# Xiaoming-Zhao/PointNav-VO

Hardware: AMD Instinct MI355X
Metric: RGB-D frame-pair VO inferences/s @341x192 (higher is better)
Workload: dtype f32

## Files before the change

### include/pnvo.h

```cpp
#ifndef PNVO_H_
#define PNVO_H_

#include <stddef.h>
#include <stdint.h>

#ifdef __cplusplus
extern "C" {
#endif

#define PNVO_OK 0
#define PNVO_ERR_ARG (-1)
#define PNVO_ERR_HIP (-2)
#define PNVO_ERR_STATE (-3)
#define PNVO_ERR_WEIGHTS (-4)
#define PNVO_ERR_INPUT (-5)

typedef struct pnvo_model_s *pnvo_handle;

typedef struct {
  int32_t width, height;
  int32_t n_rgb, n_depth, n_dd, n_tdv;
  int32_t baseplanes;
  int32_t hidden;
  int32_t out_dim;
// ... 124 lines not shown
int pnvo_policy_load_weights(pnvo_policy_handle h, const float *blob, size_t n_floats, const pnvo_tensor_desc *toc,
                             int ntoc);

int pnvo_policy_act(pnvo_policy_handle h, const float *depth, const float *goal, const int64_t *prev_actions,
                    const float *masks, const float *hidden_in, int B, float *hidden_out, float *features, float *logits,
                    float *value, void *stream);

int pnvo_policy_destroy(pnvo_policy_handle h);

int pnvo_avgpool2(const float *depth, int N, int H, int W, float *out, void *stream);

const char *pnvo_last_error(pnvo_handle h);

const char *pnvo_last_note(pnvo_handle h);


int pnvo_set_tap(pnvo_handle h, const char *name, float *dst, size_t capacity);
int pnvo_tap_shape(pnvo_handle h, const char *name, int B, int64_t shape[4]);

typedef struct {
  char name[96];
  int64_t launches;
  double total_ms;
  double flops;
  double bytes;
} pnvo_kernel_time;
int pnvo_forward_features(pnvo_handle h, const float *rgb, const float *depth, const float *dd, const float *tdv,
                          const int64_t *actions, int B, float *hidden_out, void *stream);

int pnvo_check_inputs(pnvo_handle h);

int pnvo_layer_kernel(pnvo_handle h, const char *name, int B, char *family, size_t cap, double *executed_flops);

int pnvo_timing_mode(pnvo_handle h, int mode);
int pnvo_timing_read(pnvo_handle h, pnvo_kernel_time *entries, int cap, int *n_out);

size_t pnvo_packed_conv_floats(int cout, int cin, int kh, int kw);
int pnvo_pack_conv_weight(const float *oihw, int cout, int cin, int kh, int kw, float *out);

int pnvo_resize_area(const void *src, int src_dtype, int n, int in_h, int in_w, int channels, int64_t src_frame_stride,
                     int64_t src_row_stride, int64_t src_pix_stride, int rs_h, int rs_w, int crop_y, int crop_x, int out_h, int out_w,
                     float *dst, int dst_group, int64_t dst_group_stride, int64_t dst_member_stride, int64_t dst_row_stride,
                     int64_t dst_pix_stride, int div_rule, void *stream);

const char *pnvo_version(void);

#ifdef __cplusplus
}
#endif
#endif
```

### pointnav-vo_amd/_lib.py

```python
import ctypes as C
import os

import torch

_HERE = os.path.dirname(os.path.abspath(__file__))
LIB_PATH = os.path.join(_HERE, "csrc", "libpnvo.so")

PNVO_OK = 0


GRAD_READY_FN = C.CFUNCTYPE(None, C.c_void_p, C.c_uint64, C.c_uint64, C.c_void_p)


class PnvoError(RuntimeError):
    pass


class pnvo_config(C.Structure):
    _fields_ = [(n, C.c_int32) for n in (
        "width", "height", "n_rgb", "n_depth", "n_dd", "n_tdv", "baseplanes", "hidden", "out_dim", "normalize",
        "act_embed", "n_acts", "flat_size", "max_batch", "backbone_depth")]


class pnvo_tensor_desc(C.Structure):
# ... 35 lines not shown
    "pnvo_dataset_pairs": (C.c_int, [C.c_void_p] * 7 + [C.c_int] * 5 + [C.c_void_p] * 7),
    "pnvo_topdown_view_pairs": (C.c_int, [C.c_void_p, C.c_int, C.c_int, C.c_int, C.POINTER(C.c_float), C.c_int, C.c_void_p, C.c_void_p,
                                          C.c_void_p]),
    "pnvo_topdown_view": (C.c_int, [C.c_void_p, C.c_int, C.c_int, C.c_int, C.c_int64, C.c_int64,
                                    C.POINTER(C.c_float), C.c_int, C.c_void_p, C.c_int64, C.c_int64, C.c_void_p,
                                    C.c_void_p]),
    "pnvo_train_attach": (C.c_int, [C.c_void_p, C.c_void_p, C.c_void_p, C.c_size_t, C.POINTER(pnvo_tensor_desc), C.c_int]),
    "pnvo_train_refresh": (C.c_int, [C.c_void_p, C.c_void_p]),
    "pnvo_train_forward": (C.c_int, [C.c_void_p, C.c_void_p, C.c_void_p, C.c_void_p, C.c_void_p, C.c_int, C.c_void_p,
                                     C.c_void_p, C.c_void_p, C.c_void_p]),
    "pnvo_train_backward": (C.c_int, [C.c_void_p, C.c_void_p, C.c_void_p]),
    "pnvo_train_set_grad_hook": (C.c_int, [C.c_void_p, C.c_void_p, C.c_void_p]),
    "pnvo_train_grad_buckets": (C.c_int, [C.c_void_p, C.POINTER(C.c_uint64), C.POINTER(C.c_uint64), C.c_int, C.POINTER(C.c_int)]),
    "pnvo_input_moments": (C.c_int, [C.c_void_p, C.c_void_p, C.c_void_p, C.c_void_p, C.c_void_p, C.c_int, C.c_void_p,
                                     C.c_int, C.c_void_p, C.c_void_p]),
    "pnvo_rmv_merge": (C.c_int, [C.c_void_p, C.c_int, C.c_int, C.c_void_p, C.c_void_p, C.c_void_p, C.c_void_p]),
    "pnvo_train_set_actions": (C.c_int, [C.c_void_p, C.c_void_p]),
    "pnvo_mse_loss": (C.c_int, [C.c_void_p, C.c_void_p, C.c_int, C.c_int, C.c_void_p, C.c_void_p, C.c_void_p]),
    "pnvo_mse_loss_coef": (C.c_int, [C.c_void_p, C.c_void_p, C.c_void_p, C.c_int, C.c_void_p, C.c_void_p, C.c_void_p]),
    "pnvo_geo_inverse_loss": (C.c_int, [C.c_void_p, C.c_void_p, C.c_int, C.c_int, C.c_float, C.c_void_p, C.c_void_p,
                                        C.c_void_p]),
    "pnvo_train_set_dropout": (C.c_int, [C.c_void_p, C.c_float, C.c_uint64]),
    "pnvo_train_dropout_mask": (C.c_int, [C.c_void_p, C.c_int, C.c_void_p, C.c_void_p]),
    "pnvo_adam_step": (C.c_int, [C.c_void_p, C.c_void_p, C.c_void_p, C.c_void_p, C.c_size_t, C.c_float, C.c_float,
                                 C.c_float, C.c_float, C.c_int, C.c_void_p]),
    "pnvo_destroy": (C.c_int, [C.c_void_p]),
    "pnvo_ring_assemble": (C.c_int, [C.c_void_p, C.c_void_p, C.c_void_p, C.c_void_p, C.c_void_p, C.c_void_p, C.c_void_p, C.c_int, C.c_int,
                                     C.c_int, C.c_void_p, C.c_void_p, C.c_void_p, C.c_void_p]),
    "pnvo_last_error": (C.c_char_p, [C.c_void_p]),
    "pnvo_last_note": (C.c_char_p, [C.c_void_p]),
    "pnvo_set_tap": (C.c_int, [C.c_void_p, C.c_char_p, C.c_void_p, C.c_size_t]),
    "pnvo_tap_shape": (C.c_int, [C.c_void_p, C.c_char_p, C.c_int, C.POINTER(C.c_int64)]),
    "pnvo_check_inputs": (C.c_int, [C.c_void_p]),
    "pnvo_forward_features": (C.c_int, [C.c_void_p, C.c_void_p, C.c_void_p, C.c_void_p, C.c_void_p, C.c_void_p, C.c_int,
                                        C.c_void_p, C.c_void_p]),
    "pnvo_policy_create": (C.c_int, [C.c_void_p, C.c_int, C.POINTER(C.c_void_p)]),
    "pnvo_policy_load_weights": (C.c_int, [C.c_void_p, C.c_void_p, C.c_size_t, C.c_void_p, C.c_int]),
    "pnvo_policy_act": (C.c_int, [C.c_void_p, C.c_void_p, C.c_void_p, C.c_void_p, C.c_void_p, C.c_void_p, C.c_int,
                                  C.c_void_p, C.c_void_p, C.c_void_p, C.c_void_p, C.c_void_p]),
    "pnvo_policy_destroy": (C.c_int, [C.c_void_p]),
    "pnvo_avgpool2": (C.c_int, [C.c_void_p, C.c_int, C.c_int, C.c_int, C.c_void_p, C.c_void_p]),
    "pnvo_layer_kernel": (C.c_int, [C.c_void_p, C.c_char_p, C.c_int, C.c_char_p, C.c_size_t, C.POINTER(C.c_double)]),
    "pnvo_timing_mode": (C.c_int, [C.c_void_p, C.c_int]),
    "pnvo_timing_read": (C.c_int, [C.c_void_p, C.POINTER(pnvo_kernel_time), C.c_int, C.POINTER(C.c_int)]),
    "pnvo_packed_conv_floats": (C.c_size_t, [C.c_int, C.c_int, C.c_int, C.c_int]),
    "pnvo_pack_conv_weight": (C.c_int, [C.c_void_p, C.c_int, C.c_int, C.c_int, C.c_int, C.c_void_p]),
    "pnvo_resize_area": (C.c_int, [C.c_void_p, C.c_int, C.c_int, C.c_int, C.c_int, C.c_int, C.c_int64, C.c_int64, C.c_int64,
                                   C.c_int, C.c_int, C.c_int, C.c_int, C.c_int, C.c_int, C.c_void_p, C.c_int, C.c_int64, C.c_int64,
                                   C.c_int64, C.c_int64, C.c_int, C.c_void_p]),
    "pnvo_version": (C.c_char_p, []),
}


def _load():
    if not os.path.exists(LIB_PATH):
        raise PnvoError(
            f"{LIB_PATH} is missing: the HIP extension has not been built.  Run "
            "`python -c 'import __graft_entry__ as g; g.build()'` (or `make -C pointnav-vo_amd/csrc`).  "
            "There is no CPU fallback.")
    lib = C.CDLL(LIB_PATH)
    for name, (res, args) in _SIGNATURES.items():
        fn = getattr(lib, name)
        fn.restype = res
        fn.argtypes = args
    return lib

# ... 13 lines not shown
```

### pointnav-vo_amd/csrc/pnvo_api.hip

```cpp
#include <hip/hip_runtime.h>

#include <cmath>
#include <cstdio>
#include <cstdlib>
#include <cstring>
#include <functional>
#include <atomic>
#include <condition_variable>
#include <map>
#include <mutex>
#include <string>
#include <thread>
#include <vector>

#include "pnvo_model.h"

using namespace pnvo;

thread_local std::string g_err;

int pnvo_fail(pnvo_handle h, int code, const std::string &msg) {
  if (h) h->err = msg;
  g_err = msg;
  return code;
// ... 578 lines not shown
  xa.y = r.y;
  xa.in_scale = r.in_scale;
  xa.in_shift = r.in_shift;
  xa.stats = m->stats;
  if (r.tail != nullptr) {
    if (r.in_scale == nullptr) return fail(m, PNVO_ERR_STATE, "block tail without the conv's GroupNorm scale/shift");
    xa.xout = r.tail->out;
  }
  const long P = (long)l.hout * l.wout;
  const int cpg = l.groups > 0 ? l.cout / l.groups : 0;
  const bool fuse = m->opt.gn_fuse && xa.slots == 1 && l.cout == l.coutp && cpg >= 1 && cpg <= 32 &&
                    32 % cpg == 0 && l.cout % cpg == 0 && (rows || !(xa.persist_wgs > 0 && l.cin == 32 && l.coutp == 32));
  if (fuse && ride != nullptr) {
    xa.ds_gamma = ride->cd->gamma;
    xa.ds_beta = ride->cd->beta;
    xa.ds_scale = ride->ss[0];
    xa.ds_shift = ride->ss[1];
    xa.ds_mu = ride->mu;
    xa.ds_rstd = ride->rstd;
  }
  if (fuse) {
    xa.gn_gamma = l.gamma;
    xa.gn_beta = l.beta;
    xa.gn_scale = r.ss[0];
    xa.gn_shift = r.ss[1];
    xa.gn_mu = r.mu;
    xa.gn_rstd = r.rstd;
    xa.gn_cpg = cpg;
    xa.gn_eps = 1e-5f;
    xa.gn_P = P;
  }
  {
    Timed t(m, s, "conv:" + l.name, conv_flops(l, B), conv_bytes(l, B) + (r.tail ? 8.0 * B * l.hin * l.win * l.cin : 0.0));
    if (rows)
      HIPCHK(m, launch_conv_rows32(xa, x3_mode, m->num_cus, s));
    else
      HIPCHK(m, launch_conv_x3(xa, l.k, l.stride, x3_mode, mw, nw, ldsb, s));
  }
  if (fuse) return PNVO_OK;
  Timed t(m, s, "gn_finalize", 0.0, 0.0);
  if (ride != nullptr) {
    const float *st2[2] = {m->stats, m->stats_ds}, *ga2[2] = {l.gamma, ride->cd->gamma}, *be2[2] = {l.beta, ride->cd->beta};
    float *sc2[2] = {r.ss[0], ride->ss[0]}, *sh2[2] = {r.ss[1], ride->ss[1]};
    float *mu2[2] = {r.mu, ride->mu}, *rs2[2] = {r.rstd, ride->rstd};
    HIPCHK(m, launch_gn_finalize_pair(st2, B, xa.slots, l.coutp, l.cout, l.groups, P, ga2, be2, 1e-5f, sc2, sh2, mu2, rs2, s,
                                      r.grp ? &gg : nullptr, r.grp ? &ggd : nullptr));
    return PNVO_OK;
  }
  HIPCHK(m, launch_gn_finalize(m->stats, B, xa.slots, l.coutp, l.cout, l.groups, P, 1, l.gamma, l.beta, 1e-5f, r.ss[0], r.ss[1], s,
                               xa.slots, r.mu, r.rstd, r.grp ? &gg : nullptr));
  return PNVO_OK;
}

int run_conv_fp32(pnvo_handle m, const Layer &l, int B, const ConvRequest &r) {
  hipStream_t s = r.s;
  ConvArgs a;
  conv_geometry(l, B, r.y_cstride, a);
  if (r.src != nullptr) {
    const int nsrc[4] = {m->cfg.n_rgb, m->cfg.n_depth, m->cfg.n_dd, m->cfg.n_tdv};
    a.src_mode = 1;
    a.zero_page = m->zero_page;
    for (int j = 0; j < m->CP / 8; ++j)
      for (int hh = 0; hh < 2; ++hh)
        for (int q = 0; q < 2; ++q) {
          const int nc = 8 * j + 4 * hh + 2 * q;
          const int tn = m->stem_tensor_of_new[nc];
          SrcPiece &pc = a.pieces[j][hh][q];
// ... 45 lines not shown
      a.kpart = m->kpart;
      a.ksplit = ks;
    }
  }
  {
    Timed t(m, s, "conv:" + l.name, conv_flops(l, B), conv_bytes(l, B));
    HIPCHK(m, launch_conv(a, s));
    if (a.ksplit > 1 && r.head_out != nullptr && P == 1 && r.y_cstride == l.cout) {
      HIPCHK(m, launch_ksplit_reduce_head(a, r.head_w, m->head_bias, m->cfg.out_dim, r.head_out, s));
      if (r.head_rode != nullptr) *r.head_rode = true;
    } else if (a.ksplit > 1) {
      HIPCHK(m, launch_ksplit_reduce(a, s));
    }
  }
  if (r.ss) {
    Timed t(m, s, "gn_finalize", 0.0, 0.0);
    HIPCHK(m, launch_gn_finalize(m->stats, B, a.slots, l.coutp, l.cout, l.groups, P, a.MT * 32, l.gamma, l.beta, 1e-5f,
                                 r.ss[0], r.ss[1], s, 0, r.mu, r.rstd));
  }
  return PNVO_OK;
}
}

int pnvo_run_conv(pnvo_handle m, const Layer &l, int B, const ConvRequest &r) {
  if (r.ss && r.src == nullptr && r.bias == nullptr && !r.relu_out && r.y_cstride == l.coutp && x3_layer(m, l)) {
    ConvX3Args xa;
    x3_fill(m, l, B, xa);
    if (r.tail != nullptr) {
      xa.res = r.tail->res;
      xa.res_scale = r.tail->res_scale;
      xa.res_shift = r.tail->res_shift;
    }
    const int x3_mode = r.tail ? (r.tail->res ? 2 : 3) : (r.in_scale ? 1 : 0);
    const bool rows = xa.np == 2 && m->opt.x3_rows && conv_rows32_plan(xa, l.k, l.stride, x3_mode, m->num_cus);
    int mw = 0, nw = 0;
    size_t ldsb = 0;
    if (rows || conv_x3_plan(xa, l.k, l.stride, &mw, &nw, &ldsb)) return run_conv_x3(m, l, B, r, xa, rows, x3_mode, mw, nw, ldsb);
  }
  if (r.tail != nullptr) return fail(m, PNVO_ERR_STATE, "block tail handed to a conv that cannot take it (" + l.name + ")");
  if (r.grp != nullptr && r.ss != nullptr) return fail(m, PNVO_ERR_STATE, "grouped forward: layer " + l.name + " fell off the float16-piece tile kernel");
  return run_conv_fp32(m, l, B, r);
}

StemPlan pnvo_stem_plan(pnvo_handle m, bool train_fwd, const RawFrames &raw) {
  const Layer &stem = m->convs[0];
  StemPlan p;
  p.lds_serves = (m->CPL <= 32) && (stem.coutp == 32 || stem.coutp == 64) && stem.cout == stem.coutp;
  const bool keeps_place = !m->dense_sticky || (!train_fwd && p.lds_serves);
  if (keeps_place && m->mx_ok && (!train_fwd || m->train_mx) && m->opt.stem <= 1)
    p.kernel = StemPlan::MX;
  else if (keeps_place && m->dd_ok && m->opt.stem != 3)
    p.kernel = StemPlan::DD;
  else
    p.kernel = p.lds_serves ? StemPlan::LDS : StemPlan::GENERIC;
  const bool fused = p.kernel == StemPlan::MX || p.kernel == StemPlan::DD;
  p.standin = fused && m->dense_sticky;
  p.slots = stem_slots(m, p.kernel);
  const bool on_device = m->opt.input_fallback && m->dd_flag != nullptr && !train_fwd && p.lds_serves;
  p.repairs = fused && !p.standin && raw.depth == nullptr && on_device;
  p.marks = m->dd_flag != nullptr && !m->dense_sticky && raw.depth == nullptr && !on_device;
  const bool loaded_current = m->train == nullptr || m->weights_gen == m->weights_gen_at_load;
  const bool h2_current = m->mx_wpk2_dev || (train_fwd ? m->train == nullptr : loaded_current);
  const bool want2 = train_fwd ? m->opt.train_pieces == 2 : m->opt.pieces == 2;
  p.pieces = (want2 && h2_current && m->mx_wpk2 != nullptr) ? 2 : 3;
  p.h2_from_host = m->opt.pieces == 2 && m->mx_wpk2 != nullptr && loaded_current;
  return p;
}
// ... 1530 lines not shown
    int hh = h->Hp, ww = h->Wp;
    for (int k = 1; k < li; ++k) {
      hh = halve(hh);
      ww = halve(ww);
    }
    return set(B, hh, ww, c.baseplanes << (li - 1));
  }
  return fail(h, PNVO_ERR_ARG, "unknown tap '" + n + "'");
}

int pnvo_layer_kernel(pnvo_handle h, const char *name, int B, char *family, size_t cap, double *executed_flops) {
  if (!h || !name || !family || cap == 0 || B <= 0) return fail(h, PNVO_ERR_ARG, "bad argument");
  for (size_t li = 1; li < h->convs.size(); ++li) {
    const Layer &l = h->convs[li];
    if (l.name != name) continue;
    const double alg = 2.0 * B * l.hout * l.wout * (double)l.cout * l.cin * l.k * l.kw;
    if (pnvo_stem_plan(h, false, {}).writes_slots() && pnvo_small_usable(h, B)) {
      std::snprintf(family, cap, "smallnet");
      if (executed_flops) {
        const int mb = l.cinp >= 128 ? 1 : l.cinp >= 64 ? 2 : 4, th = mb == 4 ? 8 : 4, tw = mb == 1 ? 4 : 8;
        *executed_flops = 2.0 * B * ((l.hout + th - 1) / th) * ((l.wout + tw - 1) / tw) * (th * tw) * (double)rup(l.cout, 16) * l.cinp * l.k * l.kw;
      }
      return PNVO_OK;
    }
    ConvX3Args xa;
    int mw, nw;
    size_t ldsb;
    if (l.k == 1 && l.stride == 2 && li >= 3 && h->convs[li - 2].stride == 2 && pnvo_conv_takes_ds(h, h->convs[li - 2], l, B) &&
        x3_args(h, h->convs[li - 2], B, xa, &mw, &nw, &ldsb)) {
      std::snprintf(family, cap, "x2-rides");
      if (executed_flops) *executed_flops = 3.0 * 2.0 * (double)B * xa.tiles_r * xa.tiles_c * xa.MT * 32.0 * l.coutp * (double)l.cinp;
      return PNVO_OK;
    }
    if (x3_layer(h, l) && l.groups > 0 && x3_args(h, l, B, xa, &mw, &nw, &ldsb)) {
      std::snprintf(family, cap, xa.np == 2 ? "x2" : "x3");
      if (executed_flops)
        *executed_flops = (xa.np == 2 ? 3.0 : 6.0) * 2.0 * (double)B * xa.tiles_r * xa.tiles_c * xa.MT * 32.0 * l.coutp * (double)l.cinp * l.k * l.kw;
      return PNVO_OK;
    }
    std::snprintf(family, cap, "%s", layer_on_lds(h, l, nullptr) ? "fp32-lds" : "fp32-generic");
    if (executed_flops) *executed_flops = alg;
    return PNVO_OK;
  }
  return fail(h, PNVO_ERR_ARG, std::string("no residual-stage conv named '") + name + "'");
}

int pnvo_timing_mode(pnvo_handle h, int mode) {
  if (!h) return fail(h, PNVO_ERR_ARG, "null handle");
  h->timing = mode ? 1 : 0;
  return PNVO_OK;
}

int pnvo_timing_read(pnvo_handle h, pnvo_kernel_time *entries, int cap, int *n_out) {
  if (!h || !n_out) return fail(h, PNVO_ERR_ARG, "null argument");
  for (auto &r : h->trecs) {
    HIPCHK(h, hipEventSynchronize(r.b));
    float ms = 0.f;
    HIPCHK(h, hipEventElapsedTime(&ms, r.a, r.b));
    h->tentries[r.entry].total_ms += ms;
    h->evpool.push_back(r.a);
    h->evpool.push_back(r.b);
  }
  h->trecs.clear();
  const int n = (int)h->tentries.size();
  *n_out = n;
  for (int k = 0; k < n && k < cap && entries; ++k) entries[k] = h->tentries[k];
  h->tentries.clear();
  h->tindex.clear();
  return PNVO_OK;
}

size_t pnvo_packed_conv_floats(int cout, int cin, int kh, int kw) { return packed_conv_floats(cout, cin, kh, kw); }

int pnvo_pack_conv_weight(const float *oihw, int cout, int cin, int kh, int kw, float *out) {
  if (!oihw || !out || cout <= 0 || cin <= 0 || kh <= 0 || kw <= 0) return fail(nullptr, PNVO_ERR_ARG, "bad argument");
  pack_conv_weight(oihw, cout, cin, kh, kw, out);
  return PNVO_OK;
// ... 4 lines not shown
```

### pointnav-vo_amd/csrc/pnvo_internal.h

```cpp
#pragma once
#include <mutex>
#include <hip/hip_runtime.h>
#include <stdint.h>

namespace pnvo {

constexpr int PNVO_ABSMAX_UINTS = 64 * 16;

struct SrcPiece {
  const float *base;
  int nch;
  int choff;
};

struct ConvArgs {
  const float *x;
  const float *wpk;
  float *y;
  const float *in_scale;
  const float *in_shift;
  float *stats;
  const float *bias;
  const int64_t *bias_row;
  int B, H, W, CIN;
// ... 132 lines not shown
  float *ds_scale, *ds_shift;
  float *ds_mu, *ds_rstd;
  int grp_end0, grp_end1;
  const unsigned short *wpk_g[2], *ds_wpk_g[2];
  float oscale_g[2], ds_oscale_g[2];
  const float *gn_gamma_g[2], *gn_beta_g[2], *ds_gamma_g[2], *ds_beta_g[2];
};
#if defined(__HIPCC__)
__device__ __forceinline__ void gn_finalize_lane(float s1, float s2, int cpg, long P, float eps, float gamma, float beta, float *scale, float *shift,
                                                 float *mu_out = nullptr, float *rstd_out = nullptr) {
#pragma clang fp contract(off)
  double d1 = (double)s1, d2 = (double)s2;
  for (int o = cpg >> 1; o >= 1; o >>= 1) {
    d1 += __shfl_xor(d1, o);
    d2 += __shfl_xor(d2, o);
  }
  const double cnt = (double)P * cpg;
  const double mu = d1 / cnt;
  double var = d2 / cnt - mu * mu;
  if (var < 0.0) var = 0.0;
  const double rstd = 1.0 / sqrt(var + (double)eps);
  if (mu_out != nullptr) {
    *mu_out = (float)mu;
    *rstd_out = (float)rstd;
  }
  const double sc = rstd * (double)gamma;
  *scale = (float)sc;
  *shift = (float)((double)beta - mu * sc);
}
#endif
bool conv_x3_plan(ConvX3Args &a, int ks, int stride, int *mw, int *nw, size_t *lds_bytes);
bool conv_rows32_plan(ConvX3Args &a, int ks, int stride, int mode, int num_cus);
hipError_t launch_conv_rows32(const ConvX3Args &a, int mode, int num_cus, hipStream_t s);
hipError_t launch_conv_x3(const ConvX3Args &a, int ks, int stride, int mode, int mw, int nw, size_t lds_bytes, hipStream_t s);
hipError_t launch_conv_x3_repack(const float *w_oihw, int cout, int cin, int cinp, int coutp, int kh, int kw, int transposed,
                                 unsigned short *out, hipStream_t s);
void pack_conv_x3_weight(const float *oihw, int cout, int cin, int cinp, int coutp, int kh, int kw, unsigned short *out);
hipError_t launch_conv_x2_scales(const float *params, const long *seg_dev, int nseg, float *out, hipStream_t s);
hipError_t launch_conv_x2_repack(const float *w_oihw, int cout, int cin, int cinp, int coutp, int kh, int kw, const float *scale_dev,
                                 unsigned short *out, hipStream_t s, int transposed = 0);
float pack_conv_x2_weight(const float *oihw, int cout, int cin, int cinp, int coutp, int kh, int kw, unsigned short *out);

struct ConvBArgs {
  const unsigned short *x[2];
  const unsigned short *wpk[2];
  void *y[2];
  const float *in_scale[2], *in_shift[2];
  const unsigned short *x2[2];
  const float *in_scale2[2], *in_shift2[2];
  unsigned short *xout[2];
  float *stats[2];
  int B, H, W, CIN, Ho, Wo, COUTP;
  int TR, TC, tiles_r, tiles_c, PR, PC, CK, MT, wn, slots;
  int persist_wgs;
  const unsigned short *ds_wpk[2];
  void *ds_y[2];
  float *ds_stats[2];
  const float *ds_gamma[2], *ds_beta[2];
  float *ds_scale[2], *ds_shift[2];
  const float *gn_gamma[2], *gn_beta[2];
  float *gn_scale[2], *gn_shift[2];
  int gn_cpg;
  float gn_eps;
  long gn_P;
};
bool conv_bf16_plan(ConvBArgs &a, int ks, int stride, int *mw, int *nw, size_t *lds_bytes);
// ... 200 lines not shown
```

### pointnav-vo_amd/vo_cnn.py

```python
import ctypes as C
import math

import numpy as np
import torch
import torch.nn as nn

from . import _lib
from . import model_spec as ms
from .common_vars import DEFAULT_DELTA_STATE_SIZE, N_ACTS, TOP_DOWN_VIEW_PAIR_CHANNEL
from .registry import baseline_registry


class _Holder(nn.Module):
    """Anonymous container so dotted state_dict names resolve exactly as in the reference module tree."""


def _init_tensor(name, shape, fan_in=None):
    t = torch.empty(shape)
    if len(shape) == 4 or (len(shape) == 2 and name != "action_embedding.weight"):
        if name == "output_head.1.weight":
            nn.init.orthogonal_(t)
        else:
            nn.init.kaiming_uniform_(t, a=math.sqrt(5))
    elif name == "action_embedding.weight":
# ... 244 lines not shown
            _lib.check(_lib.lib.pnvo_forward_raw(self._handle, p_rgb, p_dep, p_tdv, act_ptr, int(B), C.c_void_p(out.data_ptr()),
                                                 C.c_void_p(err_flag.data_ptr()) if err_flag is not None else None,
                                                 C.c_void_p(stream)), self._handle)
        return out

    def tap(self, name, observation_pairs, actions=None):
        dev = next(self.parameters()).device
        self._ensure_handle(dev)
        first = next(v for v in observation_pairs.values())
        B = first.shape[0]
        shape = (C.c_int64 * 4)()
        _lib.check(_lib.lib.pnvo_tap_shape(self._handle, name.encode(), int(B), shape), self._handle)
        buf = torch.empty(tuple(int(s) for s in shape), device=dev, dtype=torch.float32)
        _lib.check(_lib.lib.pnvo_set_tap(self._handle, name.encode(), C.c_void_p(buf.data_ptr()), buf.numel()),
                   self._handle)
        try:
            out = self.forward(observation_pairs, actions)
        finally:
            _lib.lib.pnvo_set_tap(self._handle, None, None, 0)
        return out, buf

    def check_inputs(self):
        if self._handle is not None:
            _lib.check(_lib.lib.pnvo_check_inputs(self._handle), self._handle)

    def layer_kernel(self, name, batch):
        dev = next(self.parameters()).device
        self._ensure_handle(dev)
        self._sync_weights()
        buf, fl = C.create_string_buffer(32), C.c_double(0.0)
        _lib.check(_lib.lib.pnvo_layer_kernel(self._handle, name.encode(), int(batch), buf, 32, C.byref(fl)), self._handle)
        return buf.value.decode(), float(fl.value)

    def timing(self, enable):
        dev = next(self.parameters()).device
        self._ensure_handle(dev)
        _lib.check(_lib.lib.pnvo_timing_mode(self._handle, int(bool(enable))), self._handle)

    def timing_read(self):
        ent = (_lib.pnvo_kernel_time * 128)()
        n = C.c_int(0)
        _lib.check(_lib.lib.pnvo_timing_read(self._handle, ent, 128, C.byref(n)), self._handle)
        return [dict(name=ent[i].name.decode(), launches=int(ent[i].launches), total_ms=float(ent[i].total_ms),
                     flops=float(ent[i].flops), bytes=float(ent[i].bytes)) for i in range(min(n.value, 128))]


def _obs_ptrs(model, observation_pairs, dev):
    c = model.cfg
    ptrs, B, keep = [], None, []
    for key, n in (("rgb", c.n_rgb), ("depth", c.n_depth), ("discretized_depth", c.n_dd), ("top_down_view", c.n_tdv)):
        if n == 0:
            ptrs.append(None)
            continue
        t = observation_pairs[key]
        if t.device != dev:
            raise RuntimeError(f"observation '{key}' is on {t.device}, model on {dev}")
        t = t.to(torch.float32).contiguous()
        if t.dim() != 4 or t.shape[1] != c.height or t.shape[2] != c.width or t.shape[3] != n:
            raise ValueError(f"observation '{key}' has shape {tuple(t.shape)}, expected [B,{c.height},{c.width},{n}]")
        B = t.shape[0] if B is None else B
        assert t.shape[0] == B
        keep.append(t)
        ptrs.append(C.c_void_p(t.data_ptr()))
    return ptrs, B, keep


# ... 146 lines not shown
```

Before: 114,300.

## Add 64-channel row-streaming MFMA conv kernel with DMA-to-LDS staging

Adds a specialized persistent row-streaming 3x3 conv kernel for 64-input-channel layers. Two wave sets alternate between MFMA compute and staging. Staging issues buffer loads directly into an LDS ring, applies GroupNorm scale/shift, ReLU and the residual, and splits values into fp16 hi/lo pairs. The dispatcher routes eligible inference layers to it instead of the 32-row kernel, and a run_layer API is added for testing single layers. It trades higher LDS use and register pressure for overlap of load, convert and compute, and applies only to inference paths without training or grouping.

New measurement: 115,400, median of 5. 1.01x the previous value.

```diff
diff --git a/include/pnvo.h b/include/pnvo.h
--- a/include/pnvo.h
+++ b/include/pnvo.h
@@ -180,6 +180,10 @@
 
 int pnvo_layer_kernel(pnvo_handle h, const char *name, int B, char *family, size_t cap, double *executed_flops);
 
+int pnvo_run_layer(pnvo_handle h, const char *name, int B, const float *x, const float *in_scale, const float *in_shift,
+                   const float *res, const float *res_scale, const float *res_shift, float *xout, float *y, float *scale,
+                   float *shift, void *stream);
+
 int pnvo_timing_mode(pnvo_handle h, int mode);
 int pnvo_timing_read(pnvo_handle h, pnvo_kernel_time *entries, int cap, int *n_out);
 
diff --git a/pointnav-vo_amd/_lib.py b/pointnav-vo_amd/_lib.py
--- a/pointnav-vo_amd/_lib.py
+++ b/pointnav-vo_amd/_lib.py
@@ -91,6 +91,7 @@
     "pnvo_set_tap": (C.c_int, [C.c_void_p, C.c_char_p, C.c_void_p, C.c_size_t]),
     "pnvo_tap_shape": (C.c_int, [C.c_void_p, C.c_char_p, C.c_int, C.POINTER(C.c_int64)]),
     "pnvo_check_inputs": (C.c_int, [C.c_void_p]),
+    "pnvo_run_layer": (C.c_int, [C.c_void_p, C.c_char_p, C.c_int] + [C.c_void_p] * 11),
     "pnvo_forward_features": (C.c_int, [C.c_void_p, C.c_void_p, C.c_void_p, C.c_void_p, C.c_void_p, C.c_void_p, C.c_int,
                                         C.c_void_p, C.c_void_p]),
     "pnvo_policy_create": (C.c_int, [C.c_void_p, C.c_int, C.POINTER(C.c_void_p)]),
diff --git a/pointnav-vo_amd/csrc/conv_rows64.hip b/pointnav-vo_amd/csrc/conv_rows64.hip
--- /dev/null
+++ b/pointnav-vo_amd/csrc/conv_rows64.hip
@@ -0,0 +1,444 @@
+#include <cstdio>
+#include <cstdlib>
+
+#include "pnvo_internal.h"
+
+namespace pnvo {
+
+typedef float f32x16 __attribute__((ext_vector_type(16)));
+typedef float f32x4 __attribute__((ext_vector_type(4)));
+typedef float f32x2 __attribute__((ext_vector_type(2)));
+typedef _Float16 f16x8 __attribute__((ext_vector_type(8)));
+typedef _Float16 f16x2 __attribute__((ext_vector_type(2)));
+typedef unsigned u32x4 __attribute__((ext_vector_type(4)));
+typedef unsigned u32x2 __attribute__((ext_vector_type(2)));
+
+#ifndef PNVO_ROWS_ABL
+#define PNVO_ROWS_ABL 0
+#endif
+#if PNVO_ROWS_ABL
+#define R6_DBG(p) ((p).rs_dbg)
+#else
+#define R6_DBG(p) 0
+#endif
+
+namespace {
+constexpr int R6_THREADS = 512;
+constexpr int R6_HG = 64;
+constexpr int R6_RING = 256;
+constexpr int R6_TAIL = 48;
+constexpr int R6_PITCH = 272;
+constexpr int R6_RAW = (R6_RING + R6_TAIL) * R6_PITCH;
+constexpr int R6_XCH = R6_RAW + 2 * 16384;
+constexpr int R6_OTAB = R6_XCH + 8 * 4096;
+constexpr int R6_MTAB = R6_OTAB + 4 * R6_HG * 4;
+constexpr int R6_SS = R6_MTAB + 4 * R6_HG * 4;
+constexpr int R6_RED = R6_SS + 256 * 4;
+constexpr int R6_DOF = R6_RED + 8 * 32 * 2 * 4;
+constexpr int R6_LDS = R6_DOF + 512 * 16;
+static_assert(R6_LDS <= 160 * 1024, "conv_rows64: LDS plan");
+
+__device__ __forceinline__ void r6_barrier() { asm volatile("s_waitcnt lgkmcnt(0)\n\ts_barrier" ::: "memory"); }
+
+__device__ __forceinline__ unsigned r6_pack2h(float a, float b) {
+  const f16x2 r = __builtin_convertvector(f32x2{a, b}, f16x2);
+  return __builtin_bit_cast(unsigned, r);
+}
+}
+
+template <int MODE>
+__global__ __launch_bounds__(R6_THREADS) __attribute__((amdgpu_waves_per_eu(2, 2))) void conv_rows64_kernel(const ConvX3Args p) {
+  extern __shared__ __attribute__((aligned(16))) unsigned char lds[];
+  const int tid = (int)threadIdx.x;
+  const int lane = tid & 63;
+  const int wave = __builtin_amdgcn_readfirstlane(tid >> 6);
+  const int set = wave >> 2, sw = wave & 3, stid = tid & 255;
+  const int nj = sw & 1, kq = sw >> 1;
+  const int H = p.H, W = p.W, P = W + 2;
+  const int dR = (2 * R6_HG) / P, dC = 2 * R6_HG - dR * P;
+
+  u32x4 bres[18][2];
+#pragma unroll
+  for (int st = 0; st < 18; ++st)
+#pragma unroll
+    for (int pc = 0; pc < 2; ++pc)
+      bres[st][pc] = *reinterpret_cast<const u32x4 *>(reinterpret_cast<const char *>(p.wpk) +
+                                                      (size_t)((((st >> 1) * 4 + 2 * kq + (st & 1)) * 2 + nj) * 2048 + pc * 1024 + lane * 16));
+  const float os = p.oscale_ptr != nullptr ? *p.oscale_ptr : p.oscale;
+  const bool res_ss = MODE == 2 && p.res_scale != nullptr;
+
+  const int q = stid & 15, jb = stid >> 4;
+  int lane_ = lane, q_ = q, jb_ = jb;
+  int tid_ = tid;
+  unsigned *otab = reinterpret_cast<unsigned *>(lds + R6_OTAB) + set * 2 * R6_HG;
+  float *mtab = reinterpret_cast<float *>(lds + R6_MTAB) + set * 2 * R6_HG;
+  float *red = reinterpret_cast<float *>(lds + R6_RED);
+  float *sstab = reinterpret_cast<float *>(lds + R6_SS);
+  const unsigned rawbase = (unsigned)(R6_RAW + set * 16384 + sw * 4096);
+  const unsigned xch_mine = (unsigned)(R6_XCH + wave * 4096 + lane * 16), xch_partner = (unsigned)(R6_XCH + (wave ^ 2) * 4096 + lane * 16);
+
+  const unsigned tbytes = (unsigned)p.B * (unsigned)(H * W * 256);
+  const __amdgpu_buffer_rsrc_t rx = __builtin_amdgcn_make_buffer_rsrc((void *)p.x, 0, tbytes, 0x00020000);
+  const __amdgpu_buffer_rsrc_t ry = __builtin_amdgcn_make_buffer_rsrc((void *)p.y, 0, tbytes, 0x00020000);
+  const __amdgpu_buffer_rsrc_t rres = __builtin_amdgcn_make_buffer_rsrc((void *)(MODE == 2 ? p.res : p.x), 0, tbytes, 0x00020000);
+  const __amdgpu_buffer_rsrc_t rxo = __builtin_amdgcn_make_buffer_rsrc((void *)(MODE == 2 ? p.xout : p.y), 0, tbytes, 0x00020000);
+
+  for (int n = (int)blockIdx.x; n < p.B; n += (int)gridDim.x) {
+    const int O0 = P;
+    const int nout = H * P;
+    const int NH = (nout + R6_HG - 1) / R6_HG;
+    const int nbase = n * H * W * 256;
+    if (tid < 128) sstab[tid] = tid < 64 ? p.in_scale[(size_t)n * 64 + tid] : p.in_shift[(size_t)n * 64 + tid - 64];
+    else if (res_ss && tid < 256) sstab[tid] = tid < 192 ? p.res_scale[(size_t)n * 64 + tid - 128] : p.res_shift[(size_t)n * 64 + tid - 192];
+    int iR, iC, iD;
+    {
+      const int f = O0 - 2 * R6_HG + R6_HG * (1 + set) + jb + 256 * P;
+      iR = f / P - 256;
+      iC = f - (iR + 256) * P;
+      iD = (((iR - 1) * W + iC - 1) * 64 + 4 * q) * 4 + nbase;
+    }
+    int oR = 0, oC = 0, oD = 0;
+    if (stid < R6_HG) {
+      const int f = O0 + R6_HG * set + stid;
+      oR = f / P;
+      oC = f - oR * P;
+      oD = ((oR - 1) * W + oC - 1) * 256 + nbase;
+    }
+
+    unsigned vok = 0, vokn = 0;
+    u32x4 *const dofp = reinterpret_cast<u32x4 *>(lds + R6_DOF) + tid;
+    auto issue = [&]() {
+      vokn = 0;
+      unsigned off[4];
+      u32x4 dn = {0, 0, 0, 0};
+#pragma unroll
+      for (int k = 0; k < 4; ++k) {
+        const int r16 = (16 * k) / P, c16 = 16 * k - r16 * P;
+        const int cw = iC + c16 >= P ? 1 : 0;
+        const int R = iR + r16 + cw, Cc = iC + c16 - cw * P;
+        const bool ok = (unsigned)(R - 1) < (unsigned)H && (unsigned)(Cc - 1) < (unsigned)W;
+        const unsigned dense = (unsigned)(iD + (16 * k - 2 * (r16 + cw)) * 256);
+        off[k] = ok ? dense - 1024u * k : 0x80000000u;
+        vokn |= ok ? (1u << k) : 0u;
+        if (MODE == 2) dn[k] = ok ? dense : 0x80000000u;
+      }
+      if (MODE == 2) *dofp = dn;
+      if (!(R6_DBG(p) & 1))
+      asm volatile(
+          "s_waitcnt lgkmcnt(0)\n\t"
+          "s_mov_b32 m0, %5\n\ts_nop 0\n\t"
+          "buffer_load_dwordx4 %0, %4, 0 offen lds\n\t"
+          "buffer_load_dwordx4 %1, %4, 0 offen offset:1024 lds\n\t"
+          "buffer_load_dwordx4 %2, %4, 0 offen offset:2048 lds\n\t"
+          "buffer_load_dwordx4 %3, %4, 0 offen offset:3072 lds"
+          ::"v"(off[0]), "v"(off[1]), "v"(off[2]), "v"(off[3]), "s"(rx), "s"(rawbase)
+          : "memory");
+      const int wrap = iC + dC >= P ? 1 : 0;
+      iC += dC - wrap * P;
+      iR += dR + wrap;
+      iD += (2 * R6_HG - 2 * (dR + wrap)) * 256;
+    };
+    f32x4 w[4];
+    u32x4 dof = {0, 0, 0, 0};
+    auto load_skip = [&]() {
+#pragma unroll
+      for (int k = 0; k < 4; ++k) w[k] = __builtin_bit_cast(f32x4, __builtin_amdgcn_raw_buffer_load_b128(rres, dof[k], 0, 0));
+      asm volatile("" ::: "memory");
+    };
+    f32x4 vk[4], sc, sh;
+    auto read_raw = [&](int pair) {
+      if (pair == 0) {
+        sc = *reinterpret_cast<const f32x4 *>(sstab + 4 * q_);
+        sh = *reinterpret_cast<const f32x4 *>(sstab + 64 + 4 * q_);
+      }
+#pragma unroll
+      for (int k = 2 * pair; k < 2 * pair + 2; ++k) vk[k] = *reinterpret_cast<const f32x4 *>(lds + rawbase + 1024 * k + 16 * lane_);
+    };
+    auto convert_store = [&](int g) {
+      if (MODE == 2) {
+        sc = *reinterpret_cast<const f32x4 *>(sstab + 4 * q_);
+        sh = *reinterpret_cast<const f32x4 *>(sstab + 64 + 4 * q_);
+      }
+      if (res_ss) {
+        const f32x4 rs = *reinterpret_cast<const f32x4 *>(sstab + 128 + 4 * q_), rt = *reinterpret_cast<const f32x4 *>(sstab + 192 + 4 * q_);
+#pragma unroll
+        for (int k = 0; k < 4; ++k)
+#pragma unroll
+          for (int e = 0; e < 4; ++e) w[k][e] = __builtin_fmaf(w[k][e], rs[e], rt[e]);
+      }
+#pragma unroll
+      for (int k = 0; k < 4; ++k) {
+        if (MODE == 1 && k == 0) {
+          read_raw(1);
+          __builtin_amdgcn_sched_barrier(0);
+        }
+        if (MODE == 2) vk[k] = *reinterpret_cast<const f32x4 *>(lds + rawbase + 1024 * k + 16 * lane_);
+        float f[4];
+        const float vmk = (float)((vok >> k) & 1u);
+#pragma unroll
+        for (int e = 0; e < 4; ++e) {
+          float x = vk[k][e];
+          if (MODE == 1) x = fmaxf(__builtin_fmaf(x, sc[e], sh[e]), 0.f) * vmk;
+          if (MODE == 2) x = fmaxf(__builtin_fmaf(x, sc[e], sh[e]) + w[k][e], 0.f) * vmk;
+          f[e] = x;
+        }
+        if (MODE == 2 && !(R6_DBG(p) & 2))
+          __builtin_amdgcn_raw_buffer_store_b128(__builtin_bit_cast(u32x4, f32x4{f[0], f[1], f[2], f[3]}), rxo, dof[k], 0, 0);
+        u32x2 hi, lo;
+#pragma unroll
+        for (int e = 0; e < 2; ++e) {
+          const float a = f[2 * e], b = f[2 * e + 1];
+          const f16x2 hh = __builtin_convertvector(f32x2{a, b}, f16x2);
+          hi[e] = __builtin_bit_cast(unsigned, hh);
+          lo[e] = r6_pack2h(a - (float)hh[0], b - (float)hh[1]);
+        }
+        const unsigned pos = (unsigned)((g & 3) * R6_HG + jb_ + 16 * k);
+        *reinterpret_cast<u32x2 *>(lds + pos * R6_PITCH + 8 * q_) = hi;
+        *reinterpret_cast<u32x2 *>(lds + pos * R6_PITCH + 128 + 8 * q_) = lo;
+        if (k < 3 && (g & 3) == 0) {
+          const unsigned mpos = pos < (unsigned)R6_TAIL ? pos + R6_RING : pos;
+          *reinterpret_cast<u32x2 *>(lds + mpos * R6_PITCH + 8 * q_) = hi;
+          *reinterpret_cast<u32x2 *>(lds + mpos * R6_PITCH + 128 + 8 * q_) = lo;
+        }
+      }
+    };
+    auto tables = [&](int hg) {
+      if (stid < R6_HG) {
+        const bool ok = (unsigned)(oR - 1) < (unsigned)H && (unsigned)(oC - 1) < (unsigned)W;
+        otab[((hg >> 1) & 1) * R6_HG + stid] = ok ? (unsigned)oD : 0x80000000u;
+        mtab[((hg >> 1) & 1) * R6_HG + stid] = ok ? os : 0.f;
+        const int wrap = oC + dC >= P ? 1 : 0;
+        oC += dC - wrap * P;
+        oR += dR + wrap;
+        oD += (2 * R6_HG - 2 * (dR + wrap)) * 256;
+      }
+    };
+
+    float t1 = 0.f, t2 = 0.f;
+    f32x16 acc;
+#pragma unroll
+    for (int r = 0; r < 16; ++r) acc[r] = 0.f;
+    auto epilogue = [&](int hg, bool conv) {
+      const int rr16 = lane_ >> 5;
+      const unsigned tb = (unsigned)(((hg >> 1) & 1) * R6_HG + 32 * kq + 4 * rr16);
+      const unsigned ch4 = (unsigned)((32 * nj + (lane_ & 31)) * 4);
+      f32x4 oth[2], msk[2];
+      u32x4 ent[2];
+      auto fetch = [&](int g4) {
+        oth[g4 & 1] = *reinterpret_cast<const f32x4 *>(lds + xch_partner + 1024 * g4);
+        ent[g4 & 1] = *reinterpret_cast<const u32x4 *>(otab + tb + 8 * g4);
+        msk[g4 & 1] = *reinterpret_cast<const f32x4 *>(mtab + tb + 8 * g4);
+      };
+      if (MODE == 1) fetch(0);
+#pragma unroll
+      for (int g4 = 0; g4 < 4; ++g4) {
+        if (MODE != 1) fetch(g4);
+        if (MODE == 1 && g4 < 3) fetch(g4 + 1);
+        else if (MODE == 1 && g4 == 3 && conv) read_raw(0);
+        if (MODE == 1 || g4 == 3) __builtin_amdgcn_sched_barrier(0);
+#pragma unroll
+        for (int e = 0; e < 4; ++e) {
+          const float x = (acc[4 * g4 + e] + oth[g4 & 1][e]) * msk[g4 & 1][e];
+          if (!(R6_DBG(p) & 2)) __builtin_amdgcn_raw_buffer_store_b32(__builtin_bit_cast(unsigned, x), ry, ent[g4 & 1][e] + ch4, 0, 0);
+          t1 += x;
+          t2 = __builtin_fmaf(x, x, t2);
+        }
+      }
+    };
+    __syncthreads();
+    issue();
+
+#if PNVO_ROWS_ABL
+    unsigned long long pc_compute = 0, pc_stage = 0, pc_bar = 0, pc_wait = 0, pc_epi = 0, pc_conv = 0;
+#endif
+    for (int h = -3; h <= NH; ++h) {
+#if PNVO_ROWS_ABL
+      const unsigned long long pt0 = __builtin_readcyclecounter();
+      unsigned long long pt1 = pt0;
+#endif
+      if ((h & 1) == set) {
+        if (h >= 0 && h < NH && !(R6_DBG(p) & 4)) {
+          asm volatile("" : "+v"(tid_));
+          const int lane_ = tid_ & 63;
+          unsigned arow[2][3];
+#pragma unroll
+          for (int mt = 0; mt < 2; ++mt)
+#pragma unroll
+            for (int kh = 0; kh < 3; ++kh)
+              arow[mt][kh] = ((((unsigned)(R6_HG * h + 2 * R6_HG + 32 * (mt ^ kq) - 1) + (unsigned)((kh - 1) * P)) & (R6_RING - 1)) + (unsigned)(lane_ & 31)) * R6_PITCH +
+                             (unsigned)((lane_ >> 5) * 16 + kq * 64);
+          f32x16 c1;
+#pragma unroll
+          for (int r = 0; r < 16; ++r) acc[r] = c1[r] = 0.f;
+          u32x4 a[2][2], an[2][2];
+#pragma unroll
+          for (int mt = 0; mt < 2; ++mt) {
+            a[mt][0] = *reinterpret_cast<const u32x4 *>(lds + arow[mt][0]);
+            a[mt][1] = *reinterpret_cast<const u32x4 *>(lds + arow[mt][0] + 128);
+          }
+#pragma unroll
+          for (int st = 0; st < 18; ++st) {
+            if (st + 1 < 18) {
+              const int nt = (st + 1) >> 1, nk = (st + 1) & 1;
+#pragma unroll
+              for (int mt = 0; mt < 2; ++mt) {
+                an[mt][0] = *reinterpret_cast<const u32x4 *>(lds + arow[mt][nt / 3] + (nt % 3) * R6_PITCH + nk * 32);
+                an[mt][1] = *reinterpret_cast<const u32x4 *>(lds + arow[mt][nt / 3] + (nt % 3) * R6_PITCH + nk * 32 + 128);
+              }
+            }
+            __builtin_amdgcn_sched_barrier(0);
+            acc = __builtin_amdgcn_mfma_f32_32x32x16_f16(__builtin_bit_cast(f16x8, a[0][1]), __builtin_bit_cast(f16x8, bres[st][0]), acc, 0, 0, 0);
+            __builtin_amdgcn_sched_barrier(0);
+            c1 = __builtin_amdgcn_mfma_f32_32x32x16_f16(__builtin_bit_cast(f16x8, a[1][1]), __builtin_bit_cast(f16x8, bres[st][0]), c1, 0, 0, 0);
+            __builtin_amdgcn_sched_barrier(0);
+            acc = __builtin_amdgcn_mfma_f32_32x32x16_f16(__builtin_bit_cast(f16x8, a[0][0]), __builtin_bit_cast(f16x8, bres[st][1]), acc, 0, 0, 0);
+            __builtin_amdgcn_sched_barrier(0);
+            c1 = __builtin_amdgcn_mfma_f32_32x32x16_f16(__builtin_bit_cast(f16x8, a[1][0]), __builtin_bit_cast(f16x8, bres[st][1]), c1, 0, 0, 0);
+            __builtin_amdgcn_sched_barrier(0);
+            acc = __builtin_amdgcn_mfma_f32_32x32x16_f16(__builtin_bit_cast(f16x8, a[0][0]), __builtin_bit_cast(f16x8, bres[st][0]), acc, 0, 0, 0);
+            __builtin_amdgcn_sched_barrier(0);
+            c1 = __builtin_amdgcn_mfma_f32_32x32x16_f16(__builtin_bit_cast(f16x8, a[1][0]), __builtin_bit_cast(f16x8, bres[st][0]), c1, 0, 0, 0);
+            __builtin_amdgcn_sched_barrier(0);
+#pragma unroll
+            for (int mt = 0; mt < 2; ++mt) {
+              a[mt][0] = an[mt][0];
+              a[mt][1] = an[mt][1];
+            }
+          }
+#pragma unroll
+          for (int g4 = 0; g4 < 4; ++g4)
+            *reinterpret_cast<f32x4 *>(lds + xch_mine + 1024 * g4) = f32x4{c1[4 * g4], c1[4 * g4 + 1], c1[4 * g4 + 2], c1[4 * g4 + 3]};
+        }
+      } else {
+        __builtin_amdgcn_s_setprio(1);
+        asm volatile("s_waitcnt vmcnt(0)" ::: "memory");
+#if PNVO_ROWS_ABL
+        pt1 = __builtin_readcyclecounter();
+        pc_wait += pt1 - pt0;
+#endif
+        asm volatile("" : "+v"(tid_));
+        lane_ = tid_ & 63;
+        q_ = tid_ & 15;
+        jb_ = (tid_ >> 4) & 15;
+        vok = vokn;
+        if (MODE == 2) {
+          dof = *dofp;
+          load_skip();
+        }
+        const bool conv = h + 4 <= NH + 2 && !(R6_DBG(p) & 8);
+        if (h >= 1) epilogue(h - 1, conv);
+        else if (MODE == 1 && conv) read_raw(0);
+#if PNVO_ROWS_ABL
+        const unsigned long long pe1 = __builtin_readcyclecounter();
+        pc_epi += pe1 - pt1;
+#endif
+        if (conv) convert_store(h + 4);
+#if PNVO_ROWS_ABL
+        const unsigned long long pe2 = __builtin_readcyclecounter();
+        pc_conv += pe2 - pe1;
+#endif
+        if (h + 6 <= NH + 2) issue();
+        if (h + 1 >= 0 && h + 1 < NH) tables(h + 1);
+        __builtin_amdgcn_s_setprio(0);
+      }
+#if PNVO_ROWS_ABL
+      const unsigned long long pt2 = __builtin_readcyclecounter();
+      if ((h & 1) == set) pc_compute += pt2 - pt0; else pc_stage += pt2 - pt1;
+#endif
+      r6_barrier();
+#if PNVO_ROWS_ABL
+      pc_bar += __builtin_readcyclecounter() - pt2;
+#endif
+    }
+#if PNVO_ROWS_ABL
+    if (p.prof != nullptr && n == 7 && lane == 0) {
+      unsigned long long *d = p.prof + wave * 8;
+      d[0] = pc_compute; d[1] = pc_stage; d[2] = pc_bar; d[3] = pc_wait; d[4] = (unsigned long long)(NH + 4); d[5] = pc_epi; d[6] = pc_conv;
+    }
+#endif
+
+    if (p.stats != nullptr) {
+      t1 += __shfl_xor(t1, 32);
+      t2 += __shfl_xor(t2, 32);
+      if (lane < 32) *reinterpret_cast<f32x2 *>(red + (wave * 32 + lane) * 2) = f32x2{t1, t2};
+      __syncthreads();
+      if (wave == 0) {
+        const int c = lane, cj = c >> 5, cc = c & 31;
+        float s1 = 0.f, s2 = 0.f;
+#pragma unroll
+        for (int k = 0; k < 4; ++k) {
+          const f32x2 o = *reinterpret_cast<const f32x2 *>(red + ((cj + 2 * k) * 32 + cc) * 2);
+          s1 += o[0];
+          s2 += o[1];
+        }
+        float *dst = p.stats + (((size_t)n * p.slots) * 64 + c) * 2;
+        dst[0] = s1;
+        dst[1] = s2;
+        if (p.gn_scale != nullptr) {
+          const bool first = p.gn_mu != nullptr && c % p.gn_cpg == 0;
+          const long gi = (long)n * (64 / p.gn_cpg) + c / p.gn_cpg;
+          gn_finalize_lane(s1, s2, p.gn_cpg, p.gn_P, p.gn_eps, p.gn_gamma[c], p.gn_beta[c], p.gn_scale + (size_t)n * 64 + c,
+                           p.gn_shift + (size_t)n * 64 + c, first ? p.gn_mu + gi : nullptr, first ? p.gn_rstd + gi : nullptr);
+        }
+      }
+    }
+    __syncthreads();
+  }
+}
+
+bool conv_rows64_plan(ConvX3Args &a, int ks, int stride, int mode, int num_cus) {
+  if (ks != 3 || stride != 1 || a.np != 2 || a.CIN != 64 || a.COUTP != 64 || a.in_absmax != nullptr) return false;
+  if ((mode != 1 && mode != 2) || (mode == 2 && a.res == nullptr)) return false;
+  if (a.Ho != a.H || a.Wo != a.W || a.W + 3 > R6_HG || a.W < 8 || a.H < 4 || (long)a.B * a.H * a.W * 256 >= (1L << 31)) return false;
+  if (a.B < num_cus || a.B < 256) return false;
+#if PNVO_ROWS_ABL
+  if (const char *e = std::getenv("PNVO_ROWS_DBG")) a.rs_dbg = std::atoi(e);
+#endif
+  a.rs_bands = 1;
+  a.rs_rows = a.H;
+  a.slots = 1;
+  return true;
+}
+
+long conv_rows64_positions(const ConvX3Args &a) { return (long)(((long)a.H * (a.W + 2) + R6_HG - 1) / R6_HG) * R6_HG; }
+
+hipError_t launch_conv_rows64(const ConvX3Args &a, int mode, int num_cus, hipStream_t s) {
+  static std::mutex attr_mu;
+  static unsigned long long attr_seen = 0;
+  if (pnvo_first_launch_on_device(attr_mu, attr_seen)) {
+    hipError_t e = hipFuncSetAttribute(reinterpret_cast<const void *>(conv_rows64_kernel<1>), hipFuncAttributeMaxDynamicSharedMemorySize, R6_LDS);
+    if (e == hipSuccess)
+      e = hipFuncSetAttribute(reinterpret_cast<const void *>(conv_rows64_kernel<2>), hipFuncAttributeMaxDynamicSharedMemorySize, R6_LDS);
+    if (e != hipSuccess) return e;
+  }
+  if (a.in_scale == nullptr || a.in_shift == nullptr || (mode == 2 && (a.res == nullptr || a.xout == nullptr))) return hipErrorInvalidValue;
+  const unsigned gx = (unsigned)(a.B < num_cus ? a.B : num_cus);
+  ConvX3Args q = a;
+#if PNVO_ROWS_ABL
+  static unsigned long long *prof = nullptr;
+  if (std::getenv("PNVO_ROWS_PROF") != nullptr) {
+    if (!prof && hipMalloc((void **)&prof, 8 * 8 * 8) != hipSuccess) return hipErrorOutOfMemory;
+    (void)hipMemsetAsync(prof, 0, 8 * 8 * 8, s);
+    q.prof = prof;
+  }
+#endif
+  if (mode == 1)
+    hipLaunchKernelGGL((conv_rows64_kernel<1>), dim3(gx), dim3(R6_THREADS), R6_LDS, s, q);
+  else if (mode == 2)
+    hipLaunchKernelGGL((conv_rows64_kernel<2>), dim3(gx), dim3(R6_THREADS), R6_LDS, s, q);
+  else
+    return hipErrorInvalidValue;
+#if PNVO_ROWS_ABL
+  if (q.prof != nullptr) {
+    unsigned long long h[64];
+    (void)hipStreamSynchronize(s);
+    (void)hipMemcpy(h, prof, sizeof(h), hipMemcpyDeviceToHost);
+    for (int w = 0; w < 8; w += 3)
+      std::fprintf(stderr, "[pnvo] conv_rows64 wave %d: per half-step (cycles): compute role %.0f  stage role %.0f = reads + epilogue %.0f | DMA issue + conversion %.0f | tables (+ wait for its loads/stores %.0f)  barrier %.0f  (%llu half-steps)\n",
+                   w, 2.0 * h[8 * w] / h[8 * w + 4], 2.0 * h[8 * w + 1] / h[8 * w + 4], 2.0 * h[8 * w + 5] / h[8 * w + 4], 2.0 * h[8 * w + 6] / h[8 * w + 4], 2.0 * h[8 * w + 3] / h[8 * w + 4], (double)h[8 * w + 2] / h[8 * w + 4], h[8 * w + 4]);
+  }
+#endif
+  return hipGetLastError();
+}
+
+}
diff --git a/pointnav-vo_amd/csrc/pnvo_api.hip b/pointnav-vo_amd/csrc/pnvo_api.hip
--- a/pointnav-vo_amd/csrc/pnvo_api.hip
+++ b/pointnav-vo_amd/csrc/pnvo_api.hip
@@ -634,7 +634,9 @@
   }
   {
     Timed t(m, s, "conv:" + l.name, conv_flops(l, B), conv_bytes(l, B) + (r.tail ? 8.0 * B * l.hin * l.win * l.cin : 0.0));
-    if (rows)
+    if (rows && xa.CIN == 64)
+      HIPCHK(m, launch_conv_rows64(xa, x3_mode, m->num_cus, s));
+    else if (rows)
       HIPCHK(m, launch_conv_rows32(xa, x3_mode, m->num_cus, s));
     else
       HIPCHK(m, launch_conv_x3(xa, l.k, l.stride, x3_mode, mw, nw, ldsb, s));
@@ -746,7 +748,10 @@
       xa.res_shift = r.tail->res_shift;
     }
     const int x3_mode = r.tail ? (r.tail->res ? 2 : 3) : (r.in_scale ? 1 : 0);
-    const bool rows = xa.np == 2 && m->opt.x3_rows && conv_rows32_plan(xa, l.k, l.stride, x3_mode, m->num_cus);
+    const bool rows64 = xa.np == 2 && m->opt.x3_rows && m->train == nullptr && r.mu == nullptr && r.grp == nullptr && r.ride == nullptr &&
+                        (r.tail == nullptr || r.tail->out != nullptr) &&
+                        conv_rows64_plan(xa, l.k, l.stride, x3_mode, m->num_cus);
+    const bool rows = rows64 || (xa.np == 2 && m->opt.x3_rows && conv_rows32_plan(xa, l.k, l.stride, x3_mode, m->num_cus));
     int mw = 0, nw = 0;
     size_t ldsb = 0;
     if (rows || conv_x3_plan(xa, l.k, l.stride, &mw, &nw, &ldsb)) return run_conv_x3(m, l, B, r, xa, rows, x3_mode, mw, nw, ldsb);
@@ -2343,6 +2348,14 @@
       if (executed_flops) *executed_flops = 3.0 * 2.0 * (double)B * xa.tiles_r * xa.tiles_c * xa.MT * 32.0 * l.coutp * (double)l.cinp;
       return PNVO_OK;
     }
+    if (x3_layer(h, l) && l.groups > 0 && h->opt.x3_rows && h->train == nullptr) {
+      x3_fill(h, l, B, xa);
+      if (xa.np == 2 && conv_rows64_plan(xa, l.k, l.stride, 1, h->num_cus)) {
+        std::snprintf(family, cap, "x2");
+        if (executed_flops) *executed_flops = 3.0 * 2.0 * (double)B * (double)conv_rows64_positions(xa) * l.coutp * (double)l.cinp * l.k * l.kw;
+        return PNVO_OK;
+      }
+    }
     if (x3_layer(h, l) && l.groups > 0 && x3_args(h, l, B, xa, &mw, &nw, &ldsb)) {
       std::snprintf(family, cap, xa.np == 2 ? "x2" : "x3");
       if (executed_flops)
@@ -2354,6 +2367,25 @@
     return PNVO_OK;
   }
   return fail(h, PNVO_ERR_ARG, std::string("no residual-stage conv named '") + name + "'");
+}
+
+int pnvo_run_layer(pnvo_handle h, const char *name, int B, const float *x, const float *in_scale, const float *in_shift, const float *res,
+                   const float *res_scale, const float *res_shift, float *xout, float *y, float *scale, float *shift, void *stream) {
+  if (!h || !name || B <= 0 || !x || !y || !scale || !shift || (in_scale == nullptr) != (in_shift == nullptr) ||
+      (res != nullptr && (in_scale == nullptr || xout == nullptr)) || (res_scale == nullptr) != (res_shift == nullptr) ||
+      (res_scale != nullptr && res == nullptr))
+    return fail(h, PNVO_ERR_ARG, "bad argument");
+  for (size_t li = 1; li < h->convs.size(); ++li) {
+    const Layer &l = h->convs[li];
+    if (l.name != name || l.groups <= 0) continue;
+    if (l.host_w.empty()) return fail(h, PNVO_ERR_STATE, "no weights loaded");
+    if (int rc = ensure_workspace(h, B)) return rc;
+    float *ss[2] = {scale, shift};
+    const BlockTail tail{res, res_scale, res_shift, xout};
+    return pnvo_run_conv(h, l, B, {.x = x, .in_scale = in_scale, .in_shift = in_shift, .y = y, .y_cstride = l.coutp, .ss = ss,
+                                   .tail = res ? &tail : nullptr, .s = (hipStream_t)stream});
+  }
+  return fail(h, PNVO_ERR_ARG, std::string("no GroupNorm-ed conv named '") + name + "'");
 }
 
 int pnvo_timing_mode(pnvo_handle h, int mode) {
diff --git a/pointnav-vo_amd/csrc/pnvo_internal.h b/pointnav-vo_amd/csrc/pnvo_internal.h
--- a/pointnav-vo_amd/csrc/pnvo_internal.h
+++ b/pointnav-vo_amd/csrc/pnvo_internal.h
@@ -188,6 +188,9 @@
 bool conv_x3_plan(ConvX3Args &a, int ks, int stride, int *mw, int *nw, size_t *lds_bytes);
 bool conv_rows32_plan(ConvX3Args &a, int ks, int stride, int mode, int num_cus);
 hipError_t launch_conv_rows32(const ConvX3Args &a, int mode, int num_cus, hipStream_t s);
+bool conv_rows64_plan(ConvX3Args &a, int ks, int stride, int mode, int num_cus);
+long conv_rows64_positions(const ConvX3Args &a);
+hipError_t launch_conv_rows64(const ConvX3Args &a, int mode, int num_cus, hipStream_t s);
 hipError_t launch_conv_x3(const ConvX3Args &a, int ks, int stride, int mode, int mw, int nw, size_t lds_bytes, hipStream_t s);
 hipError_t launch_conv_x3_repack(const float *w_oihw, int cout, int cin, int cinp, int coutp, int kh, int kw, int transposed,
                                  unsigned short *out, hipStream_t s);
diff --git a/pointnav-vo_amd/vo_cnn.py b/pointnav-vo_amd/vo_cnn.py
--- a/pointnav-vo_amd/vo_cnn.py
+++ b/pointnav-vo_amd/vo_cnn.py
@@ -300,6 +300,25 @@
         _lib.check(_lib.lib.pnvo_layer_kernel(self._handle, name.encode(), int(batch), buf, 32, C.byref(fl)), self._handle)
         return buf.value.decode(), float(fl.value)
 
+    def run_layer(self, name, x, in_scale=None, in_shift=None, res=None, res_scale=None, res_shift=None, stride=1):
+        dev = next(self.parameters()).device
+        self._ensure_handle(dev)
+        self._sync_weights()
+        B = int(x.shape[0])
+        w = self.state_dict()[name + ".weight"]
+        cout = int(w.shape[0])
+        ho, wo = (int(x.shape[1]) - 1) // stride + 1, (int(x.shape[2]) - 1) // stride + 1
+        y = torch.empty((B, ho, wo, cout), device=dev, dtype=torch.float32)
+        sc = torch.empty((B, cout), device=dev, dtype=torch.float32)
+        sh = torch.empty_like(sc)
+        xout = torch.empty_like(x) if res is not None else None
+        ts = [t.contiguous() if t is not None else None for t in (x, in_scale, in_shift, res, res_scale, res_shift)]
+        ptr = lambda t: C.c_void_p(t.data_ptr()) if t is not None else None
+        stream = torch.cuda.current_stream(dev).cuda_stream
+        _lib.check(_lib.lib.pnvo_run_layer(self._handle, name.encode(), B, *[ptr(t) for t in ts], ptr(xout), ptr(y), ptr(sc), ptr(sh),
+                                           C.c_void_p(stream)), self._handle)
+        return y, sc, sh, xout
+
     def timing(self, enable):
         dev = next(self.parameters()).device
         self._ensure_handle(dev)
```
